# lijx10/DeepI2P

Measured on AMD Instinct MI355X. Metric: frames/sec (img+pc infer + 60-restart GN pose) KITTI 20k-pt, 1/2/4/8 GPU, higher is better.
Workload: dtype f32 network (fp32-input MFMA; 3x3 convolutions, GEMM-shaped point layers and the per-point head: bf16 MFMA on exact three-way fp32 splits, fp32 accumulation) + f64 solver; 1 GPU; BASELINE configs[1]: KITTI 20480-pt / 160x512, batch 32 per GPU, coarse classification + 60-restart 2D GN/LM solver, max_iter 500; mode=frames, points=20480, restarts=60, parallelism=dp1, streams=8, hw_queues=4, hip_graph=True, weights_broadcast_bytes=0

## Files before the change

### deepi2p_amd/_lib.py

```python
import ctypes
import os

import torch

_HERE = os.path.dirname(os.path.abspath(__file__))
LIB_PATH = os.environ.get("DI2P_LIB") or os.path.join(_HERE, "lib", "libdeepi2p_hip.so")
_lib = None

c_void_p, c_int, c_float, c_double, c_ll = ctypes.c_void_p, ctypes.c_int, ctypes.c_float, ctypes.c_double, ctypes.c_longlong


class DeepI2PHipError(RuntimeError):
    pass


class SrcT(ctypes.Structure):
    _fields_ = [("ptr", c_void_p), ("gidx", c_void_p), ("batch_stride", c_ll), ("row_stride", c_int),
                ("channels", c_int), ("mode", c_int), ("group", c_int), ("pad_", c_int)]


class EpilogueT(ctypes.Structure):
    _fields_ = [("scale", c_void_p), ("shift", c_void_p), ("batch_bias", c_void_p), ("relu", c_int),
                ("group_max", c_int), ("g_table", c_void_p * 2), ("g_idx", c_void_p * 2), ("g_w", c_void_p * 2),
                ("g_nodes", c_int * 2), ("g_k", c_int * 2), ("transpose_out", c_int), ("group_max_out", c_void_p),
# ... 34 lines not shown
    "di2p_argmax_channels": [c_void_p, c_void_p, c_int, c_int, c_int, c_ll, c_void_p],
    "di2p_pointwise_gemm": [ctypes.POINTER(SrcT), c_int, c_void_p, c_void_p, c_int, c_int, c_int, c_int,
                            ctypes.POINTER(EpilogueT), c_void_p],
    "di2p_pointwise_gemm_x3": [ctypes.POINTER(SrcT), c_int, c_void_p, c_void_p, c_int, c_int, c_int, c_int,
                               ctypes.POINTER(EpilogueT), c_void_p],
    "di2p_pointwise_gemm_x3p": [c_void_p, c_void_p, c_void_p, c_int, c_int, c_int, c_int, ctypes.POINTER(EpilogueT), c_void_p],
    "di2p_bf16x3_pack": [c_void_p, c_int, c_int, c_void_p, c_void_p],
    "di2p_bf16x3_pack_conv3x3": [c_void_p, c_int, c_int, c_int, c_void_p, c_void_p],
    "di2p_batch_gemv": [c_void_p, c_int, c_int, c_void_p, c_int, c_void_p, c_int, c_void_p],
    "di2p_batch_gemv2": [c_void_p, c_int, c_int, c_void_p, c_int, c_int, c_void_p, c_int, c_void_p, c_int, c_void_p],
    "di2p_attention_pool": [c_void_p, c_void_p, c_void_p, c_int, c_int, c_int, c_int, c_void_p],
    "di2p_point_head": [c_void_p, c_int, c_void_p, c_int, c_void_p, c_void_p, c_void_p, c_void_p, c_int, c_void_p, c_void_p,
                        c_void_p, c_int, c_void_p, c_int, c_int, c_int, c_int, c_void_p],
    "di2p_point_chain": [c_void_p, c_int, c_void_p, c_int, c_void_p, c_void_p, c_void_p, c_void_p, c_int, c_void_p, c_void_p,
                         c_void_p, c_int, c_void_p, c_int, c_int, c_int, c_void_p],
    "di2p_conv2d": [c_void_p] * 6 + [c_int] * 11 + [c_void_p],
    "di2p_conv2d_ws": [c_void_p] * 6 + [c_int] * 11 + [c_void_p, c_ll, c_void_p],
    "di2p_maxpool3x3s2": [c_void_p, c_void_p, c_int, c_int, c_int, c_int, c_void_p],
    "di2p_global_avgpool": [c_void_p, c_void_p, c_int, c_int, c_int, c_void_p],
    "di2p_channel_max": [c_void_p, c_void_p, c_int, c_int, c_int, c_void_p],
    "di2p_initial_guess": [c_void_p] * 5 + [c_int, c_int, c_void_p],
    "di2p_solve_batched": [c_void_p] * 6 + [c_double, c_double, ctypes.POINTER(c_double), ctypes.POINTER(c_double)]
                          + [c_int] * 5 + [c_void_p, c_void_p, c_void_p, c_void_p, c_void_p, c_void_p],
    "di2p_solve_batched_f32": [c_void_p] * 6 + [c_double, c_double, ctypes.POINTER(c_double), ctypes.POINTER(c_double)]
                              + [c_int] * 5 + [c_void_p, c_void_p, c_void_p, c_void_p, c_void_p, c_void_p],
    "di2p_select_best": [c_void_p, c_void_p, c_void_p, c_int, c_int, c_int, c_void_p, c_void_p, c_void_p, c_void_p],
    "di2p_solver_residuals": [c_void_p] * 4 + [c_double, c_double, c_int, c_int, c_int, c_void_p, c_void_p, c_void_p, c_void_p],
    "di2p_f32_to_f64": [c_void_p, c_void_p, c_ll, c_void_p],
    "di2p_farthest_point_sampling": [c_void_p, c_void_p, c_void_p, c_void_p, c_int, c_int, c_int, c_void_p],
    "di2p_gather_points": [c_void_p, c_void_p, c_void_p, c_int, c_int, c_int, c_int, c_void_p],
# ... 216 lines not shown
```

### deepi2p_amd/csrc/common.h

```cpp
#pragma once
#include <hip/hip_runtime.h>
#include <stdint.h>
#include <stdio.h>

#include "../../include/deepi2p_hip.h"

#define DI2P_WAVE 64

void di2p_set_error(const char* fmt, ...);

#define DI2P_CHECK_ARG(cond, msg)                                   \
    do {                                                            \
        if (!(cond)) {                                              \
            di2p_set_error("%s: %s", __func__, msg);                \
            return -1;                                              \
        }                                                           \
    } while (0)

#define DI2P_RETURN_LAUNCH()                                                        \
    do {                                                                            \
        hipError_t e_ = hipGetLastError();                                          \
        if (e_ != hipSuccess) {                                                     \
            di2p_set_error("%s: launch failed: %s", __func__, hipGetErrorString(e_)); \
            return (int)e_;                                                         \
// ... 18 lines not shown
    X(SOLVER_NOCACHE, "solver_nocache", "DI2P_SOLVER_NOCACHE", 0)                  \
    X(SOLVER_PREP_SINGLE, "solver_prep_single", "DI2P_SOLVER_PREP_SINGLE", 0)      \
    X(SOLVER_PREP_BITONIC, "solver_prep_bitonic", "DI2P_SOLVER_PREP_BITONIC", 0)   \
    X(PW_X3, "pw_x3", "DI2P_PW_X3", 1)                                             \
    X(PW_NOCHAIN, "pw_nochain", "DI2P_PW_NOCHAIN", 0)                              \
    X(HEAD_REG, "head_reg", "DI2P_HEAD_REG", 0)                                    \
    X(CONV_S2SCALAR, "conv_s2scalar", "DI2P_CONV_S2SCALAR", 0)                     \
    X(CONV_X3, "conv_x3", "DI2P_CONV_X3", 31)                                      \
    X(CONV_X3_CFG, "conv_x3_cfg", "DI2P_CONV_X3_CFG", -1)                          \
    X(HEAD_X3, "head_x3", "DI2P_HEAD_X3", 1)                                       \
    X(HEAD_X3_TAB, "head_x3_tab", "DI2P_HEAD_X3_TAB", 1)                           \
    X(STEM_X3, "stem_x3", "DI2P_STEM_X3", 1)                                       \
    X(BN_UNFUSED, "bn_unfused", "DI2P_BN_UNFUSED", 0)                              \
    X(PW_X3_PLANES, "pw_x3_planes", "DI2P_PW_X3_PLANES", 1)                        \
    X(CONV_DGRAD_DENSE, "conv_dgrad_dense", "DI2P_CONV_DGRAD_DENSE", 0)            \
    X(RC_TILE64, "rc_tile64", "DI2P_RC_TILE64", 0)
enum Di2pOption {
#define DI2P_OPT_ENUM(ID, NAME, ENV, DEF) DI2P_OPT_##ID,
    DI2P_OPTIONS(DI2P_OPT_ENUM)
#undef DI2P_OPT_ENUM
    DI2P_OPT_COUNT
};
long long di2p_opt(int id);
int di2p_cu_count();
int di2p_allow_dynamic_lds(const void* kernel, size_t bytes, const char* who);
void di2p_pack_a32(const float* Wt, int K, int M, int tiles, int tile_stride, int step_stride, void* Wp, void* stream);
```

### deepi2p_amd/csrc/gemm.hip

```cpp
#include "bf16x3.h"
#include "mfma_tile.h"

#include <stdint.h>
#include <stdlib.h>

namespace {

struct LoaderWt {
    const float* Wt;
    int K, M;
    __device__ __forceinline__ float load(int k, int m) const { return (k < K && m < M) ? Wt[k * M + m] : 0.0f; }
};

struct SrcDev {
    const float* ptr[DI2P_MAX_SRC];
    const int* gidx[DI2P_MAX_SRC];
    long long batch_stride[DI2P_MAX_SRC];
    int row_stride[DI2P_MAX_SRC];
    int c_end[DI2P_MAX_SRC];
    int mode[DI2P_MAX_SRC];
    int group[DI2P_MAX_SRC];
    int n_src;
};

// ... 423 lines not shown
        if (tl.relu2) a = fmaxf(a, 0.0f);
        if (n < N) out[((long long)b * tl.P + p) * N + n] = a;
    }
}

struct ChainTail {
    const float* W1t;
    const float* sc1;
    const float* sh1;
    const float* W2t;
    const float* sc2;
    const float* sh2;
    int relu1, relu2;
};

__device__ __forceinline__ void chain_rows_to_ksteps(const float (&v)[16], float* f) {
#pragma unroll
    for (int g = 0; g < 4; ++g) {
        auto p = __builtin_amdgcn_permlane32_swap(__float_as_uint(v[4 * g + 0]), __float_as_uint(v[4 * g + 1]), false, false);
        auto q = __builtin_amdgcn_permlane32_swap(__float_as_uint(v[4 * g + 2]), __float_as_uint(v[4 * g + 3]), false, false);
        f[4 * g + 0] = __uint_as_float(p[0]);
        f[4 * g + 1] = __uint_as_float(q[0]);
        f[4 * g + 2] = __uint_as_float(p[1]);
        f[4 * g + 3] = __uint_as_float(q[1]);
    }
}

#ifndef DI2P_CHAIN_WAVES
#define DI2P_CHAIN_WAVES 2
#endif
template <int M, int KS0, int NL, int TN>
__global__ __launch_bounds__(256) __attribute__((amdgpu_waves_per_eu(DI2P_CHAIN_WAVES, 8))) void point_chain_kernel(const float* __restrict__ X, long long x_bs, int x_rs, const float* __restrict__ W0t,
                                                           int K0, EpiDev e0, ChainTail tl, float* __restrict__ Y, int N, int nblk, int total) {
    constexpr int TM = M / 32, KS = M / 2, KSMAX = KS0 > KS ? KS0 : KS;
    extern __shared__ __attribute__((aligned(16))) float lds[];
    float* w0 = lds;
    float* w1 = w0 + 2 * KS0 * M;
    float* w2 = w1 + M * M;
    float* ss = w2 + (NL == 3 ? M * M : 0);
    for (int i = threadIdx.x; i < 2 * KS0 * M; i += 256) w0[i] = i < K0 * M ? W0t[i] : 0.0f;
    for (int i = threadIdx.x; i < M * M; i += 256) w1[i] = tl.W1t[i];
    if (NL == 3)
        for (int i = threadIdx.x; i < M * M; i += 256) w2[i] = tl.W2t[i];
    {
        const float* rows[6] = {e0.scale, e0.shift, tl.sc1, tl.sh1, NL == 3 ? tl.sc2 : nullptr, NL == 3 ? tl.sh2 : nullptr};
#pragma unroll
        for (int q = 0; q < 6; ++q)
            if (rows[q] && threadIdx.x < M) ss[q * M + threadIdx.x] = rows[q][threadIdx.x];
    }
    __syncthreads();
    if (e0.scale) e0.scale = ss;
    if (e0.shift) e0.shift = ss + M;
    const int lane = threadIdx.x & 63, wave = __builtin_amdgcn_readfirstlane(threadIdx.x >> 6);
    const int l31 = lane & 31, half = lane >> 5;
// ... 3 lines not shown

    float fn[TN][KS0];
    auto request = [&](int g) {
        const int fb = g / nblk, blk = g - fb * nblk;
        const float* Xb = X + (long long)fb * x_bs;
#pragma unroll
        for (int s = 0; s < KS0; ++s) {
            const int k = 2 * s + half;
#pragma unroll
            for (int j = 0; j < TN; ++j) {
                const float x = Xb[(long long)min(k, K0 - 1) * x_rs + min((blk * TN + j) * 32 + l31, N - 1)];
                fn[j][s] = k < K0 ? x : 0.0f;
            }
        }
    };
    const int g0 = blockIdx.x * 4 + wave, stride = gridDim.x * 4;
    if (g0 < total) request(g0);
    for (int g = g0; g < total; g += stride) {
        const int b = g / nblk, blk = g - b * nblk;
        EpiPointwise ep0{e0, nullptr, b, M, N}, ep1{e1, nullptr, b, M, N}, ep2{e2, nullptr, b, M, N};
        int n[TN], nc[TN];
#pragma unroll
        for (int j = 0; j < TN; ++j) { n[j] = (blk * TN + j) * 32 + l31; nc[j] = min(n[j], N - 1); }
        float f[TN][KSMAX];
#pragma unroll
        for (int j = 0; j < TN; ++j)
#pragma unroll
            for (int s = 0; s < KS0; ++s) f[j][s] = fn[j][s];
        request(min(g + stride, total - 1));
        f32x16 acc[TM][TN];
        auto zero = [&]() {
#pragma unroll
            for (int i = 0; i < TM; ++i)
#pragma unroll
                for (int j = 0; j < TN; ++j)
#pragma unroll
                    for (int r = 0; r < 16; ++r) acc[i][j][r] = 0.0f;
        };
        auto layer = [&](const float* w, auto ks_tag) {
            constexpr int STEPS = decltype(ks_tag)::value;
            const float* wl = w + half * M + l31;
#pragma unroll
            for (int s = 0; s < STEPS; ++s) {
                float a[TM];
// ... 14 lines not shown
                    ep.apply(i * 32 + 4 * half, nc[j], acc[i][j], v);
                    chain_rows_to_ksteps(v, &f[j][i * 16]);
                }
        };
        auto to_memory = [&](const EpiPointwise& ep) {
#pragma unroll
            for (int j = 0; j < TN; ++j)
#pragma unroll
                for (int i = 0; i < TM; ++i) {
                    float v[16];
                    ep.apply(i * 32 + 4 * half, nc[j], acc[i][j], v);
                    if (n[j] < N) {
#pragma unroll
                        for (int r = 0; r < 16; ++r)
                            Y[((long long)b * M + i * 32 + 4 * half + (r & 3) + 8 * (r >> 2)) * N + n[j]] = v[r];
                    }
                }
        };
        zero();
        layer(w0, std::integral_constant<int, KS0>{});
        to_operands(ep0);
        zero();
        layer(w1, std::integral_constant<int, KS>{});
        if (NL == 3) {
            to_operands(ep1);
            zero();
            layer(w2, std::integral_constant<int, KS>{});
            to_memory(ep2);
        } else {
            to_memory(ep1);
        }
    }
}

template <bool G33, int KS0>
__global__ __launch_bounds__(512) void point_head_reg_kernel(SrcDev srcs, const float* __restrict__ W0t, int K0, EpiDev e0, HeadTail tl,
                                                              float* __restrict__ out, int N, int nblk, int total) {
    constexpr int M = HEAD_M, TM = M / 32, KS = M / 2;
    extern __shared__ __attribute__((aligned(16))) float lds[];
    float* w0 = lds;
    float* w1 = w0 + 2 * KS0 * M;
    float* w2 = w1 + M * M;
    float* ss = w2 + M * 4;
    for (int i = threadIdx.x; i < 2 * KS0 * M; i += 512) w0[i] = i < K0 * M ? W0t[i] : 0.0f;
    for (int i = threadIdx.x; i < M * M; i += 512) w1[i] = tl.W1t[i];
// ... 507 lines not shown
    PwRoute rt{};
    rt.vec = M > 64 && N % 4 == 0 && N >= 4 && M % 4 == 0 && wt_aligned && !di2p_opt(DI2P_OPT_PW_NOVEC);
    if (rt.vec) {
        rt.bm = 64; rt.bn = N % 64 != 0 ? 128 : 64; rt.bk = 32;
        rt.dense = dense;
        rt.depth = di2p_opt(DI2P_OPT_CONV_DEPTH1) == 0 && K > 2 * rt.bk ? 2 : 1;
        return rt;
    }
    rt.bn = 128; rt.bk = 16; rt.dense = 0; rt.depth = 1;
    if (M <= 32) rt.bm = 32;
    else if (M <= 64 || (long long)B * di2p_cdiv(N, 128) * di2p_cdiv(M, 128) < 256) rt.bm = 64;
    else rt.bm = 128;
    return rt;
}

struct ChainRoute { int ks0, layers, tn, nblk, wgs, w; long long total; };
static ChainRoute chain_route(int M, int K0, bool three, int B, int N, int cus) {
    ChainRoute rt{};
    rt.layers = three ? 3 : 2;
    rt.ks0 = M == 32 ? (K0 <= 8 ? 4 : 16) : (K0 <= 32 ? 16 : 32);
    rt.tn = M == 32 ? DI2P_CHAIN_TN32 : DI2P_CHAIN_TN64;
    const int wmax = M == 32 ? DI2P_CHAIN_W32 : DI2P_CHAIN_W64;
    rt.nblk = di2p_cdiv(N, 32 * rt.tn);
    rt.total = (long long)B * rt.nblk;
    rt.w = 1;
    long long best_trips = 1ll << 62;
    for (int w = wmax; w >= 1; --w) {
        const long long trips = (rt.total + 4ll * cus * w - 1) / (4ll * cus * w);
        if (trips < best_trips) { best_trips = trips; rt.w = w; }
    }
    rt.wgs = (int)std::min<long long>((long long)cus * rt.w, (rt.total + 3) / 4);
    return rt;
}

struct HeadRoute { int reg, g33, bn, nblk, wgs; long long total; };
static HeadRoute head_route(int K0, int n_src, int c0, bool reg_range, bool g33, int B, int N, int cus) {
    HeadRoute rt{};
    rt.reg = K0 <= 96 && n_src <= 2 && di2p_opt(DI2P_OPT_HEAD_REG) != 0 && (n_src != 2 || c0 % 2 == 0) && reg_range;
    rt.g33 = g33;
    rt.bn = rt.reg ? 32 : HEAD_BN;
    rt.nblk = di2p_cdiv(N, rt.bn);
    rt.total = (long long)B * rt.nblk;
    rt.wgs = rt.reg ? (int)std::min<long long>(cus, (rt.total + 7) / 8) : (int)std::min<long long>(rt.total, 1ll << 30);
    return rt;
}

// ... 45 lines not shown
            PW_CHECK(!e.planes || (!e.transpose_out && aligned16(e.planes)), "planes_out excludes transpose_out and must be 16-byte aligned");
            PW_CHECK(!e.planes || (long long)3 * M * N * 2 < (1ll << 31), "planes_out: a frame's planes must fit 31 bits");
        } else {
            PW_CHECK(!(e.g_table[0] || e.g_table[1]) || (M % 4 == 0 && M >= 4), "gathered tables need M % 4 == 0");
            PW_CHECK(!e.transpose_out || (M % 4 == 0 && e.group_max == 1), "transpose_out needs M % 4 == 0 and no group_max");
            PW_CHECK(!epi->planes_out, "planes_out: only the bf16x3 entry points write split planes");
        }
    }
    if (x3) PW_CHECK(Y || (e.planes && (e.group_max == 1 || e.gmax_out)), "Y may be NULL only when planes_out takes the full-size output");
    if (e.group_max > 1) {
        const int g = e.group_max;
        PW_CHECK((g & (g - 1)) == 0 && g <= 32 && N % g == 0, "group_max must be a power of two <= 32 dividing N");
    }
    return 0;
}
#undef PW_CHECK

extern "C" int di2p_pointwise_gemm(const di2p_src_t* srcs, int n_src, const float* Wt, float* Y, int B, int M, int K, int N,
                                   const di2p_epilogue_t* epi, void* stream) {
    DI2P_CHECK_ARG(srcs && n_src >= 1 && n_src <= DI2P_MAX_SRC, "1..3 sources");
    DI2P_CHECK_ARG(B >= 0 && M >= 1 && K >= 1 && N >= 0, "bad size");
    DI2P_CHECK_ARG((long long)K * M < (1ll << 31), "weight too large");
    if (B == 0 || N == 0) return 0;
    SrcDev s;
    bool dense;
    EpiDev e;
    if (pw_sources(__func__, srcs, n_src, K, "K", s, dense) || pw_epilogue(__func__, epi, Y, M, N, false, e)) return -1;
    hipStream_t st = (hipStream_t)stream;
    const PwRoute rt = pw_route(M, K, N, B, dense, aligned16(Wt));
    if (rt.vec) {
        if (rt.bn == 128) launch_pw_vec<TileCfg<2, 2, 1, 2, 32>>(rt.dense, rt.depth == 2, s, Wt, Y, B, M, K, N, e, st);
// ... 131 lines not shown
            hipLaunchKernelGGL((point_head_reg_kernel<false, KS0>), dim3(wgs), dim3(512), lds_reg, (hipStream_t)stream, s, W0t, K0, e, tl, out, N, nblk, (int)total);
        }
        DI2P_RETURN_LAUNCH();
    }
    const size_t lds = (HeadCfg::LDS_FLOATS + HEAD_M * HEAD_BN) * sizeof(float);
    if (rt.g33) {
        if (di2p_allow_dynamic_lds((const void*)point_head_kernel<true>, lds, __func__)) return -1;
        hipLaunchKernelGGL(point_head_kernel<true>, dim3(di2p_cdiv(N, HEAD_BN), B), dim3(HeadCfg::THREADS), lds, (hipStream_t)stream, s, W0t, K0, e, tl, out, N);
    } else {
        if (di2p_allow_dynamic_lds((const void*)point_head_kernel<false>, lds, __func__)) return -1;
        hipLaunchKernelGGL(point_head_kernel<false>, dim3(di2p_cdiv(N, HEAD_BN), B), dim3(HeadCfg::THREADS), lds, (hipStream_t)stream, s, W0t, K0, e, tl, out, N);
    }
    DI2P_RETURN_LAUNCH();
}

extern "C" int di2p_point_chain(const di2p_src_t* srcs, int n_src, const float* W0t, int K0, const di2p_epilogue_t* epi0,
                                const float* W1t, const float* scale1, const float* shift1, int relu1, const float* W2t,
                                const float* scale2, const float* shift2, int relu2, float* Y, int B, int M, int N, void* stream) {
    DI2P_CHECK_ARG(srcs && n_src == 1 && W0t && W1t && epi0, "fused chain: one dense source");
    DI2P_CHECK_ARG(M == 32 || M == 64, "fused chain: width 32 or 64 (use the separate layers otherwise)");
    DI2P_CHECK_ARG(K0 <= M, "fused chain: at most M input channels");
    DI2P_CHECK_ARG(B >= 0 && N >= 1 && K0 >= 1, "bad size");
    DI2P_CHECK_ARG(epi0->group_max <= 1 && !epi0->transpose_out && !epi0->planes_out, "fused chain: layer 0 takes scale/shift/relu/bias/gathered only");
    if (B == 0) return 0;
    DI2P_CHECK_ARG(Y && srcs[0].ptr && srcs[0].channels == K0 && srcs[0].mode == DI2P_SRC_DENSE, "fused chain: one dense source of K0 channels");
    DI2P_CHECK_ARG((long long)srcs[0].channels * srcs[0].row_stride < (1ll << 31), "per-frame source extent must fit 31 bits");
    EpiDev e;
    if (pw_epilogue(__func__, epi0, nullptr, M, N, false, e)) return -1;
    ChainTail tl{W1t, scale1, shift1, W2t, scale2, shift2, relu1, relu2};
    const float* X = srcs[0].ptr;
    const long long x_bs = srcs[0].batch_stride;
    const int x_rs = (int)srcs[0].row_stride;
    hipStream_t st = (hipStream_t)stream;
    const ChainRoute rt = chain_route(M, K0, W2t != nullptr, B, N, di2p_cu_count());
    DI2P_CHECK_ARG(rt.total < (1ll << 30), "too many column blocks");
#define DI2P_CHAIN_LAUNCH(MM, KS0, NL, TN)                                                                                          \
    do {                                                                                                                            \
        const size_t lds = (size_t)(2 * (KS0) * (MM) + ((NL) - 1) * (MM) * (MM) + 6 * (MM)) * sizeof(float);                        \
        hipLaunchKernelGGL((point_chain_kernel<MM, KS0, NL, TN>), dim3(rt.wgs), dim3(256), lds, st, X, x_bs, x_rs, W0t, K0, e, tl, Y, N, \
                           rt.nblk, (int)rt.total);                                                                                 \
    } while (0)
    const bool three = rt.layers == 3;
    if (M == 32) {
        if (rt.ks0 == 4) { if (three) DI2P_CHAIN_LAUNCH(32, 4, 3, DI2P_CHAIN_TN32); else DI2P_CHAIN_LAUNCH(32, 4, 2, DI2P_CHAIN_TN32); }
        else             { if (three) DI2P_CHAIN_LAUNCH(32, 16, 3, DI2P_CHAIN_TN32); else DI2P_CHAIN_LAUNCH(32, 16, 2, DI2P_CHAIN_TN32); }
    } else {
        if (rt.ks0 == 16) { if (three) DI2P_CHAIN_LAUNCH(64, 16, 3, DI2P_CHAIN_TN64); else DI2P_CHAIN_LAUNCH(64, 16, 2, DI2P_CHAIN_TN64); }
        else              { if (three) DI2P_CHAIN_LAUNCH(64, 32, 3, DI2P_CHAIN_TN64); else DI2P_CHAIN_LAUNCH(64, 32, 2, DI2P_CHAIN_TN64); }
    }
#undef DI2P_CHAIN_LAUNCH
    DI2P_RETURN_LAUNCH();
}

extern "C" int di2p_point_chain_route(int M, int K0, int layers, int B, int N, int cus, int32_t* out) {
    DI2P_CHECK_ARG(out && (M == 32 || M == 64) && K0 >= 1 && K0 <= M && (layers == 2 || layers == 3) && B >= 1 && N >= 1 && cus >= 1, "bad args");
    const ChainRoute rt = chain_route(M, K0, layers == 3, B, N, cus);
    DI2P_CHECK_ARG(rt.total < (1ll << 30), "too many column blocks");
    out[0] = M; out[1] = rt.ks0; out[2] = rt.layers; out[3] = rt.tn; out[4] = rt.nblk; out[5] = (int)rt.total; out[6] = rt.wgs; out[7] = rt.w;
    return 0;
}

extern "C" int di2p_point_head_route(int K0, int n_src, int c0, int reg_range, int g33, int B, int N, int cus, int32_t* out) {
    DI2P_CHECK_ARG(out && K0 >= 1 && n_src >= 1 && n_src <= DI2P_MAX_SRC && c0 >= 1 && c0 <= K0 && B >= 1 && N >= 4 && N % 4 == 0 && cus >= 1, "bad args");
    const HeadRoute rt = head_route(K0, n_src, c0, reg_range != 0, g33 != 0, B, N, cus);
    DI2P_CHECK_ARG(!rt.reg || rt.total < (1ll << 30), "too many column blocks");
    out[0] = rt.reg; out[1] = rt.g33; out[2] = rt.bn; out[3] = rt.nblk; out[4] = (int)rt.total; out[5] = rt.wgs;
    return 0;
}

extern "C" int di2p_batch_gemv(const float* Wt, int M, int k0, const float* v, int Kv, float* out, int B, void* stream) {
    DI2P_CHECK_ARG(Wt && v && out && M >= 1 && Kv >= 1 && k0 >= 0 && B >= 0, "bad args");
    if (B == 0) return 0;
    hipLaunchKernelGGL(batch_gemv_kernel, dim3(di2p_cdiv(M, 64), B), dim3(256), 0, (hipStream_t)stream, Wt, M, k0, v, Kv, 0,
// ... 21 lines not shown
```

### deepi2p_amd/networks.py

```python
import torch
import torch.nn as nn

from . import _lib, ops
from .ops import Src

BN_EPS = 1e-5


class _Holder(nn.Module):
    pass


def _register(root, key, tensor, is_buffer):
    parts = key.split(".")
    mod = root
    for p in parts[:-1]:
        if p not in mod._modules:
            mod.add_module(p, _Holder())
        mod = mod._modules[p]
    if is_buffer:
        mod.register_buffer(parts[-1], tensor)
    else:
        mod.register_parameter(parts[-1], nn.Parameter(tensor, requires_grad=False))

# ... 108 lines not shown

def _run_layer(srcs, layer, N, **kw):
    Wt, scale, shift, act = layer
    return ops.pointwise_gemm(srcs, Wt, Wt.shape[1], N, scale=scale, shift=shift, relu=act, **kw)


def _run_split_layer(dense_srcs, dense_rows, node_feats, node_rows, idx, layer, N, **kw):
    Wt, scale, shift, act = layer
    M = Wt.shape[1]
    B = node_feats.shape[0]
    G = ops.pointwise_gemm([Src(node_feats)], Wt[node_rows[0]:node_rows[1]], M, node_feats.shape[2], transpose_out=True)
    return ops.pointwise_gemm(dense_srcs, Wt[dense_rows[0]:dense_rows[1]], M, N, scale=scale, shift=shift, relu=act,
                              gathered=[(G, idx.reshape(B, N, 1), None)], **kw)


def _run_pn(x, layers, **kw):
    N = x.shape[2]
    if not kw and ops.point_chain_ok([Src(x)], layers, N):
        return ops.point_chain([Src(x)], layers, N)
    for layer in layers:
        x = _run_layer([Src(x)], layer, N, **kw)
    return x


def _run_split_pn(dense_srcs, dense_rows, node_feats, node_rows, idx, layers, N):
    Wt, scale, shift, act = layers[0]
    M = Wt.shape[1]
    B = node_feats.shape[0]
    head = (Wt[dense_rows[0]:dense_rows[1]], scale, shift, act)
    chain = [head] + list(layers[1:])
    if ops.point_chain_ok(dense_srcs, chain, N):
        G = ops.pointwise_gemm([Src(node_feats)], Wt[node_rows[0]:node_rows[1]], M, node_feats.shape[2], transpose_out=True)
        return ops.point_chain(dense_srcs, chain, N, gathered=[(G, idx.reshape(B, N, 1), None)])
    x = _run_split_layer(dense_srcs, dense_rows, node_feats, node_rows, idx, layers[0], N)
    return _run_pn(x, layers[1:])


class PCEncoder(_PackedModule):
    def __init__(self, opt, Ca: int, Cb: int, Cg: int, prefix=""):
        super().__init__()
        self.opt, self.Ca, self.Cb, self.Cg = opt, Ca, Cb, Cg
        spec = (_pn_spec("first_pointnet", 7, [Ca // 2] * 3, True)
                + _pn_spec("second_pointnet", Ca, [Ca, Ca], True)
                + _c2d_spec("knnlayer.layers_before.0", 3 + Ca, Cb) + _c2d_spec("knnlayer.layers_before.1", Cb, Cb)
                + _c2d_spec("knnlayer.layers_after.0", 2 * Cb, 2 * Cb) + _c2d_spec("knnlayer.layers_after.1", 2 * Cb, Cb)
                + _pn_spec("final_pointnet", 3 + Cb, [Cg // 2, Cg], True))
        _materialise(self, spec)

    def _pack(self):
        if self._packed is None:
# ... 10 lines not shown
        key = (B, Mb, K, str(device))
        cache = self.__dict__.setdefault("_gidx_cache", {})
        if key not in cache:
            cache[key] = (torch.arange(Mb * K, dtype=torch.int32, device=device) // K).unsqueeze(0).expand(B, -1).contiguous()
            torch.cuda.current_stream().synchronize()
        return cache[key]

    def forward_device(self, pc, intensity, sn, node_a, node_b):
        if pc.size(2) != self.opt.input_pt_num:
            raise RuntimeError("N must equal opt.input_pt_num (the reference bakes it in, networks_pc.py:44-45)")
        p = self._pack()
        B, N, Ma, Mb = pc.size(0), pc.size(2), node_a.size(2), node_b.size(2)
        idx_a, w_a = ops.knn_nodes(pc, node_a, self.opt.k_interp_point_a, want_weights=True)
        cluster_mean, mask, min_idx = ops.cluster_stats(pc, idx_a, Ma)
        pc_centers, aug = ops.build_point_input(pc, intensity, sn, cluster_mean, min_idx)
        first = _run_pn(aug, p["first"])
        _, first_max = ops.index_max(first, min_idx, Ma, return_values=True, mask=mask)
        Ch = first.shape[1]
        second = _run_split_pn([Src(first)], (0, Ch), first_max, (Ch, 2 * Ch), min_idx, p["second"], N)
        _, node_a_features = ops.index_max(second, min_idx, Ma, return_values=True, mask=mask)
        K = self.opt.k_ab
        knn_I = ops.knn_nodes(node_b, cluster_mean, K)
        coord = ops.gather_neighbors(cluster_mean, node_b, knn_I)
        y = _run_split_layer([Src(coord)], (0, 3), node_a_features, (3, 3 + node_a_features.shape[1]), knn_I.view(B, Mb * K),
                             p["layers_before.0"], Mb * K)
        pow2 = K & (K - 1) == 0 and K <= 32
        Cb1 = p["layers_before.1"][0].shape[1]
        pl = [pow2 and ops.x3_planes_link(p["layers_before.1"], p["layers_after.0"][0][Cb1:2 * Cb1], B, Mb * K),
              pow2 and ops.x3_planes_link(p["layers_after.0"], p["layers_after.1"][0], B, Mb * K)]
        if pow2:
            y, fmax = _run_layer([Src(y)], p["layers_before.1"], Mb * K, group_max=K, also_full=True, planes_out=pl[0])
            Cb = y.shape[1]
        else:
            y = _run_layer([Src(y)], p["layers_before.1"], Mb * K)
            Cb = y.shape[1]
# ... 324 lines not shown
```

### deepi2p_amd/ops.py

```python
import ctypes
import weakref

import torch

from . import _lib
from ._lib import EpilogueT, SrcT, call, ptr, require_cuda, stream

_f32, _i32, _f64 = torch.float32, torch.int32, torch.float64
MAX_GK = 16


def _chk(t, dtype, name):
    if t.dtype != dtype:
        raise RuntimeError("%s must be %s, got %s" % (name, dtype, t.dtype))


def _work(name, macs):
    if _lib.WORK is not None:
        _lib.WORK[name] = _lib.WORK.get(name, 0) + macs


def index_max(data, index, K, return_values=False, mask=None):
    require_cuda(data, index, mask)
    _chk(data, _f32, "data")
# ... 454 lines not shown
    call("di2p_point_head_labels_x3", ctypes.byref(h), B, N, stream())
    return coarse, fine


def point_chain_ok(srcs, layers, N):
    if len(layers) not in (2, 3) or len(srcs) != 1 or _lib.get_option("pw_nochain"):
        return False
    M = layers[0][0].shape[1]
    if M not in (32, 64) or layers[0][0].shape[0] > M or any(tuple(l[0].shape) != (M, M) for l in layers[1:]):
        return False
    if any(l[0].requires_grad or not l[0].is_contiguous() for l in layers):
        return False
    return srcs[0].mode == _lib.SRC_DENSE and srcs[0].t.stride(2) == 1


def point_chain(srcs, layers, N, batch_bias=None, gathered=None):
    Wt0, sc0, sh0, act0 = layers[0]
    Wt1, sc1, sh1, act1 = layers[1]
    Wt2, sc2, sh2, act2 = layers[2] if len(layers) == 3 else (None, None, None, False)
    B = srcs[0].t.shape[0]
    M = Wt0.shape[1]
    require_cuda(Wt0, Wt1, Wt2, sc0, sh0, sc1, sh1, sc2, sh2, batch_bias)
    e = EpilogueT()
    e.scale, e.shift, e.batch_bias = ptr(sc0), ptr(sh0), ptr(batch_bias)
    e.relu, e.group_max, e.transpose_out = int(bool(act0)), 1, 0
    _fill_gathered(e, gathered, B, M, N)
    out = torch.empty((B, M, N), dtype=_f32, device=Wt0.device)
    _work("di2p_point_chain", B * N * (Wt0.shape[0] * M + (len(layers) - 1) * M * M))
    call("di2p_point_chain", _fill_srcs(srcs), len(srcs), ptr(Wt0), Wt0.shape[0], ctypes.byref(e), ptr(Wt1), ptr(sc1), ptr(sh1),
         int(bool(act1)), ptr(Wt2), ptr(sc2), ptr(sh2), int(bool(act2)), ptr(out), B, M, N, stream())
    return out


def batch_gemv(Wt, k0, v):
    require_cuda(Wt, v)
    B, Kv = v.shape
    M = Wt.shape[1]
    out = torch.empty((B, M), dtype=_f32, device=Wt.device)
    call("di2p_batch_gemv", ptr(Wt), M, int(k0), ptr(v), Kv, ptr(out), B, stream())
    return out


def batch_gemv2(Wt, k0, v0, k1, v1):
    require_cuda(Wt, v0, v1)
    B = v0.shape[0]
    M = Wt.shape[1]
# ... 85 lines not shown

def rc_vec_ok(ptr, ld, batch_stride, R):
    return bool(_lib.load().di2p_rc_vec_ok(ptr, int(ld), int(batch_stride), int(R)))


def rc_route(kind, Z, rows, cols, R, a_vec=False, b_vec=False):
    out = (ctypes.c_int32 * len(RC_ROUTE_FIELDS))()
    _lib.call("di2p_rc_route", RC_KINDS.index(kind), int(Z), int(rows), int(cols), int(R), int(bool(a_vec)), int(bool(b_vec)), out)
    return dict(zip(RC_ROUTE_FIELDS, (int(v) for v in out)))


PW_ROUTE_FIELDS = ("vec", "bm", "bn", "dense", "depth", "bk")
CONV2D_ROUTE_FIELDS = ("kernel", "bm", "bn", "bk", "variant", "depth", "splits")
CONV2D_KERNELS = ("scalar", "vec", "stem_row")
WINO_ROUTE_FIELDS = ("reg", "cob", "kc", "waves", "n_tb", "tiles", "n_cb", "grid")
CHAIN_ROUTE_FIELDS = ("M", "ks0", "layers", "tn", "nblk", "total", "wgs", "w")
HEAD_ROUTE_FIELDS = ("reg", "g33", "bn", "nblk", "total", "wgs")


def _route(name, fields, *args):
    out = (ctypes.c_int32 * len(fields))()
    _lib.call(name, *(int(a) for a in args), out)
    return dict(zip(fields, (int(v) for v in out)))


def pointwise_route(M, K, N, B=1, dense=True, wt_aligned=True):
    return _route("di2p_pointwise_route", PW_ROUTE_FIELDS, M, K, N, B, bool(dense), bool(wt_aligned))


def conv2d_route(x_shape, Cout, KH, KW, stride, pad, tap_major=False, x_aligned=True, wt_aligned=True, workspace_bytes=0):
    B, Cin, H, W = x_shape
# ... 313 lines not shown
```

### include/deepi2p_hip.h

```cpp
#ifndef DEEPI2P_HIP_H
#define DEEPI2P_HIP_H

#include <stdint.h>

#ifdef __cplusplus
extern "C" {
#endif

const char* di2p_last_error(void);
int di2p_version(void);
int di2p_set_option(const char* name, long long value);
long long di2p_get_option(const char* name);

int di2p_index_max_forward(const float* data, const int32_t* index, int32_t* max_idx,
                           int B, int C, int N, int K, void* workspace, void* stream);
int di2p_index_max_values(const float* data, const int32_t* index, const float* mask, float* max_val,
                          int32_t* max_idx, int B, int C, int N, int K, void* workspace, void* stream);

int di2p_ball_query_forward(const float* node_to_point_dist, int32_t* out_idx, float radius, int K,
                            int B, int M, int N, void* stream);

int di2p_knn_nodes(const float* query, const float* nodes, int32_t* idx, float* weights,
                   int B, int Nq, int M, int k, void* stream);
int di2p_cluster_stats(const float* pc, const int32_t* knn_idx, int idx_stride, float* cluster_mean,
// ... 46 lines not shown
int di2p_bf16x3_pack_conv3x3(const float* W, int Cout, int Cin, int dgrad, void* Wp, void* stream);
int di2p_pointwise_gemm_x3(const di2p_src_t* srcs_host, int n_src, const void* Wp, float* Y,
                           int B, int M, int K, int N, const di2p_epilogue_t* epi_host, void* stream);
long long di2p_bf16x3_planes_bytes(int B, int C, int N);
int di2p_pointwise_gemm_x3p(const void* planes, const void* Wp, float* Y,
                            int B, int M, int K, int N, const di2p_epilogue_t* epi_host, void* stream);

int di2p_point_head(const di2p_src_t* srcs_host, int n_src, const float* W0t, int K0, const di2p_epilogue_t* epi0_host,
                    const float* W1t, const float* scale1, const float* shift1, int relu1,
                    const float* W2t, const float* scale2, const float* shift2, int relu2,
                    float* out, int B, int M, int P, int N, void* stream);

int di2p_point_chain(const di2p_src_t* srcs_host, int n_src, const float* W0t, int K0, const di2p_epilogue_t* epi0_host,
                     const float* W1t, const float* scale1, const float* shift1, int relu1, const float* W2t,
                     const float* scale2, const float* shift2, int relu2, float* Y, int B, int M, int N, void* stream);

int di2p_batch_gemv(const float* Wt, int M, int k0, const float* v, int Kv, float* out, int B, void* stream);
int di2p_batch_gemv2(const float* Wt, int M, int k0, const float* v0, int Kv0, int k1, const float* v1, int Kv1,
                     float* out, int B, void* stream);

int di2p_attention_pool(const float* feat, const float* score, float* out, int B, int C, int HW, int Mn, void* stream);

int di2p_conv2d(const float* x, const float* Wt, const float* scale, const float* shift,
                const float* residual, float* y, int B, int Cin, int H, int W, int Cout,
                int KH, int KW, int stride, int pad, int relu, int tap_major, void* stream);
int di2p_conv2d_ws(const float* x, const float* Wt, const float* scale, const float* shift,
                   const float* residual, float* y, int B, int Cin, int H, int W, int Cout,
                   int KH, int KW, int stride, int pad, int relu, int tap_major,
                   void* workspace, long long workspace_bytes, void* stream);
long long di2p_conv2d_workspace_bytes(int B, int Cin, int H, int W, int Cout, int KH, int KW, int stride, int pad,
// ... 263 lines not shown
```

Measured before the change: 5040 frames/s.

## Fuse per-node segment max into the point chain kernel via LDS atomic tables

Adds a segmax variant of the fused point-chain kernel. It keeps a per-block LDS table of per-node channel maxima, updated with order-preserving integer atomicMax, and flushes the table to a compact partials buffer per frame. The separate index_max pass over the full B×M×N output then runs only over the much smaller partials. The cost is LDS atomics, a changed frame-major work schedule with per-frame block barriers, and an extra partials allocation, with possible load imbalance.

```diff
diff --git a/deepi2p_amd/_lib.py b/deepi2p_amd/_lib.py
--- a/deepi2p_amd/_lib.py
+++ b/deepi2p_amd/_lib.py
@@ -72,6 +72,8 @@
                         c_void_p, c_int, c_void_p, c_int, c_int, c_int, c_int, c_void_p],
     "di2p_point_chain": [c_void_p, c_int, c_void_p, c_int, c_void_p, c_void_p, c_void_p, c_void_p, c_int, c_void_p, c_void_p,
                          c_void_p, c_int, c_void_p, c_int, c_int, c_int, c_void_p],
+    "di2p_point_chain_segmax": [c_void_p, c_int, c_void_p, c_int, c_void_p, c_void_p, c_void_p, c_void_p, c_int, c_void_p, c_void_p,
+                                c_void_p, c_int, c_void_p, c_int, c_int, c_int, c_void_p, c_int, c_int, c_void_p, c_void_p, c_void_p],
     "di2p_conv2d": [c_void_p] * 6 + [c_int] * 11 + [c_void_p],
     "di2p_conv2d_ws": [c_void_p] * 6 + [c_int] * 11 + [c_void_p, c_ll, c_void_p],
     "di2p_maxpool3x3s2": [c_void_p, c_void_p, c_int, c_int, c_int, c_int, c_void_p],
diff --git a/deepi2p_amd/csrc/common.h b/deepi2p_amd/csrc/common.h
--- a/deepi2p_amd/csrc/common.h
+++ b/deepi2p_amd/csrc/common.h
@@ -56,7 +56,8 @@
     X(BN_UNFUSED, "bn_unfused", "DI2P_BN_UNFUSED", 0)                              \
     X(PW_X3_PLANES, "pw_x3_planes", "DI2P_PW_X3_PLANES", 1)                        \
     X(CONV_DGRAD_DENSE, "conv_dgrad_dense", "DI2P_CONV_DGRAD_DENSE", 0)            \
-    X(RC_TILE64, "rc_tile64", "DI2P_RC_TILE64", 0)
+    X(RC_TILE64, "rc_tile64", "DI2P_RC_TILE64", 0)                                 \
+    X(CHAIN_SEGMAX, "chain_segmax", "DI2P_CHAIN_SEGMAX", 1)
 enum Di2pOption {
 #define DI2P_OPT_ENUM(ID, NAME, ENV, DEF) DI2P_OPT_##ID,
     DI2P_OPTIONS(DI2P_OPT_ENUM)
diff --git a/deepi2p_amd/csrc/gemm.hip b/deepi2p_amd/csrc/gemm.hip
--- a/deepi2p_amd/csrc/gemm.hip
+++ b/deepi2p_amd/csrc/gemm.hip
@@ -461,6 +461,15 @@
     int relu1, relu2;
 };
 
+struct ChainSeg {
+    const int* index;
+    float* partials;
+    int* pindex;
+    int K, parts, np;
+    int ng, frames;
+};
+constexpr unsigned kSegFloor = 0x3B85FFFFu;
+
 __device__ __forceinline__ void chain_rows_to_ksteps(const float (&v)[16], float* f) {
 #pragma unroll
     for (int g = 0; g < 4; ++g) {
@@ -476,15 +485,18 @@
 #ifndef DI2P_CHAIN_WAVES
 #define DI2P_CHAIN_WAVES 2
 #endif
-template <int M, int KS0, int NL, int TN>
+template <int M, int KS0, int NL, int TN, bool SEG>
 __global__ __launch_bounds__(256) __attribute__((amdgpu_waves_per_eu(DI2P_CHAIN_WAVES, 8))) void point_chain_kernel(const float* __restrict__ X, long long x_bs, int x_rs, const float* __restrict__ W0t,
-                                                           int K0, EpiDev e0, ChainTail tl, float* __restrict__ Y, int N, int nblk, int total) {
+                                                           int K0, EpiDev e0, ChainTail tl, float* __restrict__ Y, int N, int nblk, int total, ChainSeg sg) {
     constexpr int TM = M / 32, KS = M / 2, KSMAX = KS0 > KS ? KS0 : KS;
     extern __shared__ __attribute__((aligned(16))) float lds[];
     float* w0 = lds;
     float* w1 = w0 + 2 * KS0 * M;
     float* w2 = w1 + M * M;
     float* ss = w2 + (NL == 3 ? M * M : 0);
+    unsigned* table = reinterpret_cast<unsigned*>(ss + 6 * M);
+    if (SEG)
+        for (int i = threadIdx.x; i < M * sg.K; i += 256) table[i] = kSegFloor;
     for (int i = threadIdx.x; i < 2 * KS0 * M; i += 256) w0[i] = i < K0 * M ? W0t[i] : 0.0f;
     for (int i = threadIdx.x; i < M * M; i += 256) w1[i] = tl.W1t[i];
     if (NL == 3)
@@ -518,20 +530,23 @@
             }
         }
     };
-    const int g0 = blockIdx.x * 4 + wave, stride = gridDim.x * 4;
-    if (g0 < total) request(g0);
-    for (int g = g0; g < total; g += stride) {
+    auto block = [&](int g, int g_next) {
         const int b = g / nblk, blk = g - b * nblk;
         EpiPointwise ep0{e0, nullptr, b, M, N}, ep1{e1, nullptr, b, M, N}, ep2{e2, nullptr, b, M, N};
         int n[TN], nc[TN];
 #pragma unroll
         for (int j = 0; j < TN; ++j) { n[j] = (blk * TN + j) * 32 + l31; nc[j] = min(n[j], N - 1); }
+        int node[TN];
+        if (SEG) {
+#pragma unroll
+            for (int j = 0; j < TN; ++j) node[j] = sg.index[(long long)b * N + nc[j]];
+        }
         float f[TN][KSMAX];
 #pragma unroll
         for (int j = 0; j < TN; ++j)
 #pragma unroll
             for (int s = 0; s < KS0; ++s) f[j][s] = fn[j][s];
-        request(min(g + stride, total - 1));
+        request(g_next);
         f32x16 acc[TM][TN];
         auto zero = [&]() {
 #pragma unroll
@@ -576,6 +591,29 @@
 #pragma unroll
                         for (int r = 0; r < 16; ++r)
                             Y[((long long)b * M + i * 32 + 4 * half + (r & 3) + 8 * (r >> 2)) * N + n[j]] = v[r];
+                        if (SEG) {
+                            {
+                                const bool node_ok = (unsigned)node[j] < (unsigned)sg.K;
+                                unsigned* col = table + (i * 32 + 4 * half) * sg.K + (node_ok ? node[j] : 0);
+#pragma unroll
+                                for (int r = 0; r < 16; ++r) {
+                                    const unsigned u = __float_as_uint(v[r] + 0.0f);
+                                    const unsigned key = (u & 0x80000000u) ? ~u : (u | 0x80000000u);
+                                    atomicMax(col + ((r & 3) + 8 * (r >> 2)) * sg.K, node_ok && v[r] > -1000.0f ? key : 0u);
+                                }
+                            }
+                            if (n[j] == 0) {
+#pragma unroll
+                                for (int r = 0; r < 16; ++r) {
+                                    float* ph = sg.partials + ((long long)b * M + i * 32 + 4 * half + (r & 3) + 8 * (r >> 2)) * sg.np;
+                                    ph[0] = v[r]; ph[1] = -1000.0f; ph[2] = -1000.0f; ph[3] = -1000.0f;
+                                }
+                                if (i == 0 && half == 0) {
+                                    int* ih = sg.pindex + (long long)b * sg.np;
+                                    ih[0] = (unsigned)node[j] < (unsigned)sg.K ? node[j] : 0; ih[1] = 0; ih[2] = 0; ih[3] = 0;
+                                }
+                            }
+                        }
                     }
                 }
         };
@@ -591,6 +629,60 @@
             to_memory(ep2);
         } else {
             to_memory(ep1);
+        }
+    };
+    if constexpr (!SEG) {
+        const int g0 = blockIdx.x * 4 + wave, stride = gridDim.x * 4;
+        if (g0 < total) request(g0);
+        for (int g = g0; g < total; g += stride) block(g, min(g + stride, total - 1));
+    } else {
+        const int K = sg.K, np = sg.np, T = sg.parts, s = blockIdx.x % T, fr = gridDim.x / T;
+        auto advance = [&](int& b, int& q) {
+            do {
+                q += T;
+                if (q >= sg.ng) { q = s; b += fr; }
+            } while (b < sg.frames && q * 4 + wave >= nblk);
+        };
+        {
+            int b = blockIdx.x / T, q = s - T;
+            advance(b, q);
+            if (b < sg.frames) request(b * nblk + q * 4 + wave);
+        }
+        for (int b = blockIdx.x / T; b < sg.frames; b += fr) {
+            for (int q = s; q < sg.ng; q += T) {
+                if (q * 4 + wave >= nblk) continue;
+                const int g = b * nblk + q * 4 + wave;
+                int bn = b, qn = q;
+                advance(bn, qn);
+                block(g, bn < sg.frames ? bn * nblk + qn * 4 + wave : g);
+            }
+            __syncthreads();
+            float* pb = sg.partials + (long long)b * M * np + 4 + s * K;
+            int* ib = sg.pindex + (long long)b * np + 4 + s * K;
+            auto value = [](unsigned o) { return __uint_as_float((o & 0x80000000u) ? (o & 0x7FFFFFFFu) : ~o); };
+            if (K % 4 == 0) {
+                const int K4 = K >> 2, dm = 256 / K4, dk = 256 - dm * K4;
+                int m = (int)threadIdx.x / K4, k = (int)threadIdx.x - m * K4;
+                for (int i = threadIdx.x; i < M * K4; i += 256) {
+                    const uint4 o = reinterpret_cast<uint4*>(table)[i];
+                    reinterpret_cast<uint4*>(table)[i] = make_uint4(kSegFloor, kSegFloor, kSegFloor, kSegFloor);
+                    *reinterpret_cast<float4*>(pb + (long long)m * np + 4 * k) = make_float4(value(o.x), value(o.y), value(o.z), value(o.w));
+                    m += dm; k += dk;
+                    if (k >= K4) { k -= K4; ++m; }
+                }
+            } else {
+                const int dm = 256 / K, dk = 256 - dm * K;
+                int m = (int)threadIdx.x / K, k = (int)threadIdx.x - m * K;
+                for (int i = threadIdx.x; i < M * K; i += 256) {
+                    const unsigned o = table[i];
+                    table[i] = kSegFloor;
+                    pb[(long long)m * np + k] = value(o);
+                    m += dm; k += dk;
+                    if (k >= K) { k -= K; ++m; }
+                }
+            }
+            for (int k = threadIdx.x; k < K; k += 256) ib[k] = k;
+            __syncthreads();
         }
     }
 }
@@ -1128,7 +1220,7 @@
     return rt;
 }
 
-struct ChainRoute { int ks0, layers, tn, nblk, wgs, w; long long total; };
+struct ChainRoute { int ks0, layers, tn, nblk, wgs, w; long long total; int ng, seg_wgs, parts; };
 static ChainRoute chain_route(int M, int K0, bool three, int B, int N, int cus) {
     ChainRoute rt{};
     rt.layers = three ? 3 : 2;
@@ -1144,6 +1236,10 @@
         if (trips < best_trips) { best_trips = trips; rt.w = w; }
     }
     rt.wgs = (int)std::min<long long>((long long)cus * rt.w, (rt.total + 3) / 4);
+    rt.ng = di2p_cdiv(rt.nblk, 4);
+    const long long cap = (long long)cus * rt.w;
+    rt.parts = (int)std::max<long long>(1, std::min<long long>(cap / B, rt.ng));
+    rt.seg_wgs = rt.parts * (int)std::min<long long>(B, std::max<long long>(1, cap / rt.parts));
     return rt;
 }
 
@@ -1219,7 +1315,6 @@
     }
     return 0;
 }
-#undef PW_CHECK
 
 extern "C" int di2p_pointwise_gemm(const di2p_src_t* srcs, int n_src, const float* Wt, float* Y, int B, int M, int K, int N,
                                    const di2p_epilogue_t* epi, void* stream) {
@@ -1381,31 +1476,46 @@
     DI2P_RETURN_LAUNCH();
 }
 
-extern "C" int di2p_point_chain(const di2p_src_t* srcs, int n_src, const float* W0t, int K0, const di2p_epilogue_t* epi0,
-                                const float* W1t, const float* scale1, const float* shift1, int relu1, const float* W2t,
-                                const float* scale2, const float* shift2, int relu2, float* Y, int B, int M, int N, void* stream) {
-    DI2P_CHECK_ARG(srcs && n_src == 1 && W0t && W1t && epi0, "fused chain: one dense source");
-    DI2P_CHECK_ARG(M == 32 || M == 64, "fused chain: width 32 or 64 (use the separate layers otherwise)");
-    DI2P_CHECK_ARG(K0 <= M, "fused chain: at most M input channels");
-    DI2P_CHECK_ARG(B >= 0 && N >= 1 && K0 >= 1, "bad size");
-    DI2P_CHECK_ARG(epi0->group_max <= 1 && !epi0->transpose_out && !epi0->planes_out, "fused chain: layer 0 takes scale/shift/relu/bias/gathered only");
+static int point_chain_launch(const char* who, const di2p_src_t* srcs, int n_src, const float* W0t, int K0, const di2p_epilogue_t* epi0,
+                              const float* W1t, const float* scale1, const float* shift1, int relu1, const float* W2t,
+                              const float* scale2, const float* shift2, int relu2, float* Y, int B, int M, int N,
+                              const int32_t* seg_index, int K, int parts, float* partials, int32_t* part_index, void* stream) {
+    PW_CHECK(srcs && n_src == 1 && W0t && W1t && epi0, "fused chain: one dense source");
+    PW_CHECK(M == 32 || M == 64, "fused chain: width 32 or 64 (use the separate layers otherwise)");
+    PW_CHECK(K0 <= M, "fused chain: at most M input channels");
+    PW_CHECK(B >= 0 && N >= 1 && K0 >= 1, "bad size");
+    PW_CHECK(epi0->group_max <= 1 && !epi0->transpose_out && !epi0->planes_out, "fused chain: layer 0 takes scale/shift/relu/bias/gathered only");
     if (B == 0) return 0;
-    DI2P_CHECK_ARG(Y && srcs[0].ptr && srcs[0].channels == K0 && srcs[0].mode == DI2P_SRC_DENSE, "fused chain: one dense source of K0 channels");
-    DI2P_CHECK_ARG((long long)srcs[0].channels * srcs[0].row_stride < (1ll << 31), "per-frame source extent must fit 31 bits");
+    PW_CHECK(Y && srcs[0].ptr && srcs[0].channels == K0 && srcs[0].mode == DI2P_SRC_DENSE, "fused chain: one dense source of K0 channels");
+    PW_CHECK((long long)srcs[0].channels * srcs[0].row_stride < (1ll << 31), "per-frame source extent must fit 31 bits");
     EpiDev e;
-    if (pw_epilogue(__func__, epi0, nullptr, M, N, false, e)) return -1;
+    if (pw_epilogue(who, epi0, nullptr, M, N, false, e)) return -1;
     ChainTail tl{W1t, scale1, shift1, W2t, scale2, shift2, relu1, relu2};
     const float* X = srcs[0].ptr;
     const long long x_bs = srcs[0].batch_stride;
     const int x_rs = (int)srcs[0].row_stride;
     hipStream_t st = (hipStream_t)stream;
     const ChainRoute rt = chain_route(M, K0, W2t != nullptr, B, N, di2p_cu_count());
-    DI2P_CHECK_ARG(rt.total < (1ll << 30), "too many column blocks");
+    PW_CHECK(rt.total < (1ll << 30), "too many column blocks");
+    const bool seg = seg_index != nullptr;
+    ChainSeg sg{};
+    if (seg) {
+        PW_CHECK(partials && part_index && K >= 1 && (long long)M * K <= 8192, "segment max: partials, part_index and 1 <= K <= 8192 / M nodes");
+        PW_CHECK(parts == rt.parts, "segment max: parts must be what di2p_point_chain_route reports for this shape on this device");
+        PW_CHECK(4 + (long long)parts * K < (1ll << 24), "segment max: row of partials too long");
+        sg = ChainSeg{seg_index, partials, part_index, K, parts, 4 + parts * K, rt.ng, B};
+    }
+#define DI2P_CHAIN_LAUNCH_(MM, KS0, NL, TN, SEG)                                                                                    \
+    do {                                                                                                                            \
+        const size_t lds = (size_t)(2 * (KS0) * (MM) + ((NL) - 1) * (MM) * (MM) + 6 * (MM) + ((SEG) ? (MM) * K : 0)) * sizeof(float); \
+        if (lds > 64 * 1024 && di2p_allow_dynamic_lds((const void*)point_chain_kernel<MM, KS0, NL, TN, SEG>, lds, who)) return -1;  \
+        hipLaunchKernelGGL((point_chain_kernel<MM, KS0, NL, TN, SEG>), dim3((SEG) ? rt.seg_wgs : rt.wgs), dim3(256), lds, st, X, x_bs, x_rs, W0t, K0, e, \
+                           tl, Y, N, rt.nblk, (int)rt.total, sg);                                                                   \
+    } while (0)
 #define DI2P_CHAIN_LAUNCH(MM, KS0, NL, TN)                                                                                          \
     do {                                                                                                                            \
-        const size_t lds = (size_t)(2 * (KS0) * (MM) + ((NL) - 1) * (MM) * (MM) + 6 * (MM)) * sizeof(float);                        \
-        hipLaunchKernelGGL((point_chain_kernel<MM, KS0, NL, TN>), dim3(rt.wgs), dim3(256), lds, st, X, x_bs, x_rs, W0t, K0, e, tl, Y, N, \
-                           rt.nblk, (int)rt.total);                                                                                 \
+        if (seg) DI2P_CHAIN_LAUNCH_(MM, KS0, NL, TN, true);                                                                         \
+        else DI2P_CHAIN_LAUNCH_(MM, KS0, NL, TN, false);                                                                            \
     } while (0)
     const bool three = rt.layers == 3;
     if (M == 32) {
@@ -1416,14 +1526,35 @@
         else              { if (three) DI2P_CHAIN_LAUNCH(64, 32, 3, DI2P_CHAIN_TN64); else DI2P_CHAIN_LAUNCH(64, 32, 2, DI2P_CHAIN_TN64); }
     }
 #undef DI2P_CHAIN_LAUNCH
-    DI2P_RETURN_LAUNCH();
-}
+#undef DI2P_CHAIN_LAUNCH_
+    const hipError_t le = hipGetLastError();
+    if (le != hipSuccess) { di2p_set_error("%s: launch failed: %s", who, hipGetErrorString(le)); return (int)le; }
+    return 0;
+}
+
+extern "C" int di2p_point_chain(const di2p_src_t* srcs, int n_src, const float* W0t, int K0, const di2p_epilogue_t* epi0,
+                                const float* W1t, const float* scale1, const float* shift1, int relu1, const float* W2t,
+                                const float* scale2, const float* shift2, int relu2, float* Y, int B, int M, int N, void* stream) {
+    return point_chain_launch(__func__, srcs, n_src, W0t, K0, epi0, W1t, scale1, shift1, relu1, W2t, scale2, shift2, relu2, Y, B, M, N,
+                              nullptr, 0, 0, nullptr, nullptr, stream);
+}
+
+extern "C" int di2p_point_chain_segmax(const di2p_src_t* srcs, int n_src, const float* W0t, int K0, const di2p_epilogue_t* epi0,
+                                       const float* W1t, const float* scale1, const float* shift1, int relu1, const float* W2t,
+                                       const float* scale2, const float* shift2, int relu2, float* Y, int B, int M, int N,
+                                       const int32_t* index, int K, int parts, float* partials, int32_t* part_index, void* stream) {
+    DI2P_CHECK_ARG(index || B == 0, "segment max: index is required");
+    return point_chain_launch(__func__, srcs, n_src, W0t, K0, epi0, W1t, scale1, shift1, relu1, W2t, scale2, shift2, relu2, Y, B, M, N,
+                              index, K, parts, partials, part_index, stream);
+}
+
+#undef PW_CHECK
 
 extern "C" int di2p_point_chain_route(int M, int K0, int layers, int B, int N, int cus, int32_t* out) {
-    DI2P_CHECK_ARG(out && (M == 32 || M == 64) && K0 >= 1 && K0 <= M && (layers == 2 || layers == 3) && B >= 1 && N >= 1 && cus >= 1, "bad args");
-    const ChainRoute rt = chain_route(M, K0, layers == 3, B, N, cus);
+    DI2P_CHECK_ARG(out && (M == 32 || M == 64) && K0 >= 1 && K0 <= M && (layers == 2 || layers == 3) && B >= 1 && N >= 1 && cus >= 0, "bad args");
+    const ChainRoute rt = chain_route(M, K0, layers == 3, B, N, cus ? cus : di2p_cu_count());
     DI2P_CHECK_ARG(rt.total < (1ll << 30), "too many column blocks");
-    out[0] = M; out[1] = rt.ks0; out[2] = rt.layers; out[3] = rt.tn; out[4] = rt.nblk; out[5] = (int)rt.total; out[6] = rt.wgs; out[7] = rt.w;
+    out[0] = M; out[1] = rt.ks0; out[2] = rt.layers; out[3] = rt.tn; out[4] = rt.nblk; out[5] = (int)rt.total; out[6] = rt.wgs; out[7] = rt.w; out[8] = rt.parts; out[9] = rt.seg_wgs;
     return 0;
 }
 
diff --git a/deepi2p_amd/networks.py b/deepi2p_amd/networks.py
--- a/deepi2p_amd/networks.py
+++ b/deepi2p_amd/networks.py
@@ -146,16 +146,24 @@
                               gathered=[(G, idx.reshape(B, N, 1), None)], **kw)
 
 
-def _run_pn(x, layers, **kw):
+def _run_pn(x, layers, segmax=None, **kw):
     N = x.shape[2]
     if not kw and ops.point_chain_ok([Src(x)], layers, N):
-        return ops.point_chain([Src(x)], layers, N)
-    for layer in layers:
-        x = _run_layer([Src(x)], layer, N, **kw)
-    return x
-
-
-def _run_split_pn(dense_srcs, dense_rows, node_feats, node_rows, idx, layers, N):
+        if segmax is not None and ops.point_chain_segmax_ok(layers[0][0].shape[1], segmax[1]):
+            return ops.point_chain([Src(x)], layers, N, segmax=segmax)
+        x = ops.point_chain([Src(x)], layers, N)
+    else:
+        for layer in layers:
+            x = _run_layer([Src(x)], layer, N, **kw)
+    return x if segmax is None else (x, _segment_max(x, segmax))
+
+
+def _segment_max(x, segmax):
+    index, K, mask = segmax
+    return ops.index_max(x, index, K, return_values=True, mask=mask)[1]
+
+
+def _run_split_pn(dense_srcs, dense_rows, node_feats, node_rows, idx, layers, N, segmax=None):
     Wt, scale, shift, act = layers[0]
     M = Wt.shape[1]
     B = node_feats.shape[0]
@@ -163,9 +171,12 @@
     chain = [head] + list(layers[1:])
     if ops.point_chain_ok(dense_srcs, chain, N):
         G = ops.pointwise_gemm([Src(node_feats)], Wt[node_rows[0]:node_rows[1]], M, node_feats.shape[2], transpose_out=True)
-        return ops.point_chain(dense_srcs, chain, N, gathered=[(G, idx.reshape(B, N, 1), None)])
+        if segmax is not None and not ops.point_chain_segmax_ok(M, segmax[1]):
+            x = ops.point_chain(dense_srcs, chain, N, gathered=[(G, idx.reshape(B, N, 1), None)])
+            return x, _segment_max(x, segmax)
+        return ops.point_chain(dense_srcs, chain, N, gathered=[(G, idx.reshape(B, N, 1), None)], segmax=segmax)
     x = _run_split_layer(dense_srcs, dense_rows, node_feats, node_rows, idx, layers[0], N)
-    return _run_pn(x, layers[1:])
+    return _run_pn(x, layers[1:], segmax=segmax)
 
 
 class PCEncoder(_PackedModule):
@@ -206,11 +217,10 @@
         idx_a, w_a = ops.knn_nodes(pc, node_a, self.opt.k_interp_point_a, want_weights=True)
         cluster_mean, mask, min_idx = ops.cluster_stats(pc, idx_a, Ma)
         pc_centers, aug = ops.build_point_input(pc, intensity, sn, cluster_mean, min_idx)
-        first = _run_pn(aug, p["first"])
-        _, first_max = ops.index_max(first, min_idx, Ma, return_values=True, mask=mask)
+        first, first_max = _run_pn(aug, p["first"], segmax=(min_idx, Ma, mask))
         Ch = first.shape[1]
-        second = _run_split_pn([Src(first)], (0, Ch), first_max, (Ch, 2 * Ch), min_idx, p["second"], N)
-        _, node_a_features = ops.index_max(second, min_idx, Ma, return_values=True, mask=mask)
+        second, node_a_features = _run_split_pn([Src(first)], (0, Ch), first_max, (Ch, 2 * Ch), min_idx, p["second"], N,
+                                                segmax=(min_idx, Ma, mask))
         K = self.opt.k_ab
         knn_I = ops.knn_nodes(node_b, cluster_mean, K)
         coord = ops.gather_neighbors(cluster_mean, node_b, knn_I)
diff --git a/deepi2p_amd/ops.py b/deepi2p_amd/ops.py
--- a/deepi2p_amd/ops.py
+++ b/deepi2p_amd/ops.py
@@ -492,7 +492,15 @@
     return srcs[0].mode == _lib.SRC_DENSE and srcs[0].t.stride(2) == 1
 
 
-def point_chain(srcs, layers, N, batch_bias=None, gathered=None):
+def point_chain_segmax_ok(M, K):
+    return int(M) * int(K) <= 8192 and bool(_lib.get_option("chain_segmax"))
+
+
+def point_chain_segmax_cols(parts, K):
+    return 4 + int(parts) * int(K)
+
+
+def point_chain(srcs, layers, N, batch_bias=None, gathered=None, segmax=None):
     Wt0, sc0, sh0, act0 = layers[0]
     Wt1, sc1, sh1, act1 = layers[1]
     Wt2, sc2, sh2, act2 = layers[2] if len(layers) == 3 else (None, None, None, False)
@@ -505,9 +513,26 @@
     _fill_gathered(e, gathered, B, M, N)
     out = torch.empty((B, M, N), dtype=_f32, device=Wt0.device)
     _work("di2p_point_chain", B * N * (Wt0.shape[0] * M + (len(layers) - 1) * M * M))
-    call("di2p_point_chain", _fill_srcs(srcs), len(srcs), ptr(Wt0), Wt0.shape[0], ctypes.byref(e), ptr(Wt1), ptr(sc1), ptr(sh1),
-         int(bool(act1)), ptr(Wt2), ptr(sc2), ptr(sh2), int(bool(act2)), ptr(out), B, M, N, stream())
-    return out
+    args = (_fill_srcs(srcs), len(srcs), ptr(Wt0), Wt0.shape[0], ctypes.byref(e), ptr(Wt1), ptr(sc1), ptr(sh1),
+            int(bool(act1)), ptr(Wt2), ptr(sc2), ptr(sh2), int(bool(act2)), ptr(out), B, M, N)
+    if segmax is None:
+        call("di2p_point_chain", *args, stream())
+        return out
+    index, K, mask = segmax
+    K = int(K)
+    require_cuda(index, mask)
+    _chk(index, _i32, "segmax index")
+    if tuple(index.shape) != (B, N) or not point_chain_segmax_ok(M, K):
+        raise RuntimeError("point_chain segmax: index must be i32[B, N] and point_chain_segmax_ok(M, K) hold")
+    if B == 0:
+        return out, torch.empty((0, M, K), dtype=_f32, device=out.device)
+    parts = point_chain_route(M, Wt0.shape[0], len(layers), B, N, 0)["parts"]
+    cols = point_chain_segmax_cols(parts, K)
+    partials = torch.empty((B, M, cols), dtype=_f32, device=out.device)
+    part_index = torch.empty((B, cols), dtype=_i32, device=out.device)
+    call("di2p_point_chain_segmax", *args, ptr(index), K, parts, ptr(partials), ptr(part_index), stream())
+    _, val = index_max(partials, part_index, K, return_values=True, mask=mask)
+    return out, val
 
 
 def batch_gemv(Wt, k0, v):
@@ -623,7 +648,7 @@
 CONV2D_ROUTE_FIELDS = ("kernel", "bm", "bn", "bk", "variant", "depth", "splits")
 CONV2D_KERNELS = ("scalar", "vec", "stem_row")
 WINO_ROUTE_FIELDS = ("reg", "cob", "kc", "waves", "n_tb", "tiles", "n_cb", "grid")
-CHAIN_ROUTE_FIELDS = ("M", "ks0", "layers", "tn", "nblk", "total", "wgs", "w")
+CHAIN_ROUTE_FIELDS = ("M", "ks0", "layers", "tn", "nblk", "total", "wgs", "w", "parts", "seg_wgs")
 HEAD_ROUTE_FIELDS = ("reg", "g33", "bn", "nblk", "total", "wgs")
 
 
diff --git a/include/deepi2p_hip.h b/include/deepi2p_hip.h
--- a/include/deepi2p_hip.h
+++ b/include/deepi2p_hip.h
@@ -84,6 +84,10 @@
 int di2p_point_chain(const di2p_src_t* srcs_host, int n_src, const float* W0t, int K0, const di2p_epilogue_t* epi0_host,
                      const float* W1t, const float* scale1, const float* shift1, int relu1, const float* W2t,
                      const float* scale2, const float* shift2, int relu2, float* Y, int B, int M, int N, void* stream);
+int di2p_point_chain_segmax(const di2p_src_t* srcs_host, int n_src, const float* W0t, int K0, const di2p_epilogue_t* epi0_host,
+                            const float* W1t, const float* scale1, const float* shift1, int relu1, const float* W2t,
+                            const float* scale2, const float* shift2, int relu2, float* Y, int B, int M, int N,
+                            const int32_t* index, int K, int parts, float* partials, int32_t* part_index, void* stream);
 
 int di2p_batch_gemv(const float* Wt, int M, int k0, const float* v, int Kv, float* out, int B, void* stream);
 int di2p_batch_gemv2(const float* Wt, int M, int k0, const float* v0, int Kv0, int k1, const float* v1, int Kv1,
```

After: 5089 frames/s, median of 6. Within noise of the previous version (+1.0%).
